# hku-mars/ImMesh

Hardware: AMD Instinct MI355X
Metric: scans/sec (reg+mesh), 100k-pt scan into 10M-voxel map (higher is better)
Workload: dtype f64

## Files before the change

### immesh_amd/csrc/c_api.cpp

```cpp
#include "host_ctx.hpp"
#include "imu_host.hpp"
#include <cmath>
#include <new>

#define RP_ABORTED 1
static thread_local std::string g_create_error;
thread_local KProf* g_kprof = nullptr;



extern "C" {

void immesh_default_config(immesh_config* c) {
    std::memset(c, 0, sizeof(*c));
    c->voxel_size = 0.5; c->max_layer = 2;
    for (int i = 0; i < 5; i++) c->layer_init[i] = 5;
    c->max_points_size = 100; c->planer_threshold = 0.01; c->dept_err = 0.02; c->beam_err = 0.05; c->calib_laser = 0;
    c->sigma_num = 3.0; c->max_iter = 4;
    c->extR[0] = c->extR[4] = c->extR[8] = 1.0;
    c->extT[0] = 0.04165; c->extT[1] = 0.02326; c->extT[2] = -0.0284;
    c->mesh_min_spacing = 0.1; c->mesh_voxel = 0.4; c->mesh_region = 10.0; c->mesh_append_budget = 10000;
}

const char* immesh_create_error(void) { return g_create_error.c_str(); }
// ... 195 lines not shown
        if (rc) { c->err = "all-reduce callback failed"; return IMMESH_E_INVAL; }
    }
    c->cnt.n_match += (int64_t)c->h_out48[RES_N_MATCH];
    c->cnt.n_plane_tests += (int64_t)c->h_out48[RES_PLANE_TESTS];
    c->cnt.n_extra_probe += (int64_t)c->h_out48[RES_EXTRA_PROBE];
    return 0;
}

static int fetch_matches(immesh_ctx* c, int n, std::vector<int8_t>& mt) {
    mt.resize(n);
    HIPCHK(c, hipMemcpyAsync(mt.data(), c->d_match, n, hipMemcpyDeviceToHost, c->stream));
    HIPCHK(c, hipStreamSynchronize(c->stream));
    return 0;
}

static int register_enqueue_chain(immesh_ctx* c, const float* d_pts, int n_ds, const imh::State& st) {
    RegIterArgs& a = c->reg_args;
    const int max_iter = c->cfg.max_iter;
    for (int it = 0; it < max_iter; it++) {
        a.it = it; a.mode = REG_MODE_SUMS;
        if (it == 0) {
            double p11[36];
            for (int r = 0; r < 6; r++) for (int q = 0; q < 6; q++) p11[r * 6 + q] = st.cov[r * 18 + q];
            if (!imh::invert(p11, a.mat, 6)) return singular_prior(c);
            for (int i = 0; i < 12; i++)
                for (int q = 0; q < 6; q++) { double sacc = 0; for (int k = 0; k < 6; k++) sacc += st.cov[(6 + i) * 18 + k] * a.mat[k * 6 + q]; a.mat[36 + i * 6 + q] = sacc; }
        }
        else if (it == 1) std::memcpy(a.mat, st.cov, sizeof(a.mat));
        launch_residual(c->stream, c->map, a, c->d_regstate, d_pts, n_ds, c->d_partials, c->d_done, c->d_out48, c->d_reg_out_host, c->reg_ticket, c->d_match, c->d_mnode,
                        c->d_dis, c->d_rinv, c->d_normal);
        if (c->rccl_comm) {
            const int rc = rccl_allreduce_f64(c, c->d_out48, RES_NV - 2, c->stream);
            if (rc) return rc;
        }
        launch_ekf_step(c->stream, a, c->d_regstate, c->d_out48, c->d_reg_out_host, c->reg_ticket);
    }
    return 0;
}
static int register_enqueue_fused(immesh_ctx* c, const float* d_pts, int n_ds, const imh::State& prior, const imh::State& st, const RpEpilogue* ep = nullptr) {
    const int max_iter = c->cfg.max_iter;
    RegIterArgs& a = c->reg_args;
    make_scan_params(c, st, st.cov, a.sp);
    a.max_iter = max_iter; a.pad = 0;
    if (c->tail_deferred && !c->rccl_comm) { a.pad = 1; c->tail_deferred = false; }
    else if (c->tail_deferred) { launch_map_update_tail(c->stream, c->map, c->d_counters_host); c->tail_deferred = false; }
    std::memcpy(a.st, st.R, 72); std::memcpy(a.st + 9, st.t, 24); std::memcpy(a.st + 12, st.vel, 24); std::memcpy(a.st + 15, st.bg, 24); std::memcpy(a.st + 18, st.ba, 24); std::memcpy(a.st + 21, st.g, 24);
    std::memcpy(a.prior, prior.R, 72); std::memcpy(a.prior + 9, prior.t, 24); std::memcpy(a.prior + 12, prior.vel, 24); std::memcpy(a.prior + 15, prior.bg, 24);
    std::memcpy(a.prior + 18, prior.ba, 24); std::memcpy(a.prior + 21, prior.g, 24);
    c->reg_ticket = (double)(++c->res_ticket);
    if (!c->rccl_comm) {
        a.mode = REG_MODE_FUSED; a.it = 0;
        if (c->knobs.rp_force_abort) a.pad |= 2;
        if (c->knobs.match_seq) a.pad |= 4;
        std::memcpy(a.mat, st.cov, sizeof(a.mat));
        const int par = (c->rp_parity ^= 1);
        RpEpilogue none{};
        launch_residual_persistent(c->stream, c->map, a, c->d_regstate, d_pts, n_ds, c->d_rp_slots[par], c->d_rp_slots[par ^ 1], c->d_counters_host, c->d_reg_out_host, c->reg_ticket, c->d_match, c->d_mnode,
                                   c->d_dis, c->d_rinv, c->d_normal, ep ? *ep : none, c->rp_max_blocks);
        return 0;
    }
    return register_enqueue_chain(c, d_pts, n_ds, st);
}
static int register_collect_fused(immesh_ctx* c, int n_ds, imh::State& st, int* n_iter, int* n_match, double* res_mean) {
    volatile double* flag = c->h_reg_out + REG_OUT_TICKET;
    const double ticket = c->reg_ticket;
    bool held;
    if (const int rc = wait_pinned(c, c->stream, [&] { return *flag == ticket; }, std::chrono::milliseconds(500), WAIT_NO_YIELD, &held)) return rc;
    if (c->prof.on) HIPCHK(c, hipStreamSynchronize(c->stream));
    if (!held) { c->err = "registration kernels did not complete"; return IMMESH_E_HIP; }
    const double* o = c->h_reg_out;
    if (o[REG_OUT_PASSES] < 0) return RP_ABORTED;
    imh::load_state(o + REG_OUT_STATE, st);
    const int iters = (int)o[REG_OUT_PASSES];
    if (n_iter) *n_iter = iters;
    if (n_match) *n_match = (int)o[REG_OUT_N_MATCH];
    if (res_mean) *res_mean = o[REG_OUT_N_MATCH] > 0 ? o[REG_OUT_SUM_DIS] / o[REG_OUT_N_MATCH] : 0.0;
    c->cnt.n_match += (int64_t)o[REG_OUT_N_MATCH_SUM];
    c->cnt.n_plane_tests += (int64_t)o[REG_OUT_PLANE_TESTS];
    c->cnt.n_extra_probe += (int64_t)o[REG_OUT_EXTRA_PROBE];
    c->cnt.n_iter += iters;
    c->cnt.n_ds = n_ds;
    c->last_n_ds = n_ds;
    return 0;
}
static int register_fallback_chain(immesh_ctx* c, const float* d_pts, int n_ds, const imh::State& st) {
    HIPCHK(c, hipStreamSynchronize(c->stream));
    c->rp_fallbacks++;
    c->reg_args.pad = 0;
    c->reg_ticket = (double)(++c->res_ticket);
    return register_enqueue_chain(c, d_pts, n_ds, st);
}
static bool use_fused_ekf(const immesh_ctx* c) {
    return !c->knobs.host_ekf && !c->allreduce && c->cfg.max_iter >= 2 && c->cfg.max_iter < 62 && (c->cfg.shard_world <= 1 || c->rccl_comm != nullptr);
}

static int register_device(immesh_ctx* c, const float* d_pts, int n_ds, const imh::State& prior, imh::State& st, int* n_iter, int* n_match, double* res_mean) {
    c->last_reg_pts = d_pts;
    if (use_fused_ekf(c)) {
        int rc = register_enqueue_fused(c, d_pts, n_ds, prior, st);
        if (rc) return rc;
        rc = register_collect_fused(c, n_ds, st, n_iter, n_match, res_mean);
        if (rc != RP_ABORTED) return rc;
        if ((rc = register_fallback_chain(c, d_pts, n_ds, st))) return rc;
        return register_collect_fused(c, n_ds, st, n_iter, n_match, res_mean);
    }
    imh::EkfLoop ekf;
// ... 336 lines not shown
    if (rc) return rc;
    for (int i = 0; i < 4; i++) ms[i] = c->timing[i];
    return 0;
}

int immesh_dump_planes(immesh_ctx* c, immesh_plane_rec* out, int64_t cap, int64_t* n_out) {
    if (!c || !n_out) return IMMESH_E_INVAL;
    (void)hipSetDevice(c->cfg.device);
    ProfBind _pb(c);
    if (const int s_rc = settle(c)) return s_rc;
    static_assert(sizeof(PlaneRecDev) == sizeof(immesh_plane_rec), "plane record layout");
    PlaneRecDev* d_out = nullptr;
    if (out && cap > 0) HIPCHK(c, hipMalloc((void**)&d_out, (size_t)cap * sizeof(PlaneRecDev)));
    launch_dump_planes(c->stream, c->map, d_out, d_out ? cap : 0, c->d_dump_count);
    unsigned long long cnt = 0;
    hipError_t e = hipMemcpyAsync(&cnt, c->d_dump_count, sizeof(cnt), hipMemcpyDeviceToHost, c->stream);
    if (e == hipSuccess) e = hipStreamSynchronize(c->stream);
    if (e == hipSuccess && d_out) e = hipMemcpy(out, d_out, (size_t)std::min<int64_t>(cap, (int64_t)cnt) * sizeof(PlaneRecDev), hipMemcpyDeviceToHost);
    if (d_out) (void)hipFree(d_out);
    if (e != hipSuccess) { c->err = std::string("dump_planes: ") + hipGetErrorString(e); return IMMESH_E_HIP; }
    *n_out = (int64_t)cnt;
    return 0;
}


int immesh_counters(immesh_ctx* c, immesh_counters_t* out, int32_t reset) {
    if (!c || !out) return IMMESH_E_INVAL;
    (void)hipSetDevice(c->cfg.device);
    ProfBind _pb(c);
    if (const int s_rc = settle(c)) return s_rc;
    int64_t stats[STATS_WORDS];
    HIPCHK(c, hipMemcpyAsync(stats, c->d_stats, sizeof(stats), hipMemcpyDeviceToHost, c->stream));
    HIPCHK(c, hipMemcpyAsync(c->h_counters, c->map.counters, 16 * sizeof(int32_t), hipMemcpyDeviceToHost, c->stream));
    HIPCHK(c, hipStreamSynchronize(c->stream));
    for (int k = 0; k < 64; k++) { stats[0] += stats[16 + k * 16]; stats[1] += stats[16 + k * 16 + 1]; }
    *out = c->cnt;
    out->n_refits = stats[0]; out->n_refit_pts = stats[1];
    out->n_root_voxels = c->h_counters[6]; out->n_nodes = c->h_counters[0];
    mesh_counters(c, out);
    if (c->reg_dbg) {
        unsigned long long t[64];
        HIPCHK(c, hipMemcpy(t, c->reg_dbg, sizeof(t), hipMemcpyDeviceToHost));
        if (!c->knobs.trace_file.empty()) {
            std::vector<unsigned long long> all(REG_DBG_WORDS);
            HIPCHK(c, hipMemcpy(all.data(), c->reg_dbg, all.size() * 8, hipMemcpyDeviceToHost));
            if (FILE* f = fopen(c->knobs.trace_file.c_str(), "wb")) { fwrite(all.data(), 8, all.size(), f); fclose(f); }
        }
        HIPCHK(c, hipMemset(c->reg_dbg, 0, sizeof(t)));
        fprintf(stderr, "[replay_list] slowest fast-path voxel %llu cycles (%llu pts), slowest general voxel %llu cycles (%llu pts); mean cycles fast %llu (%llu voxels) general %llu (%llu voxels); list gather + sort %llu per voxel\n",
                t[8] >> 16, t[8] & 0xFFFF, t[9] >> 16, t[9] & 0xFFFF, t[10] / std::max(1ull, t[12]), t[12], t[11] / std::max(1ull, t[13]), t[13], t[14] / std::max(1ull, t[12] + t[13]));
        const unsigned long long nwv = std::max(1ull, t[6]), npass = std::max(1ull, t[7]);
        fprintf(stderr, "[residual cycles of wavefront 0, %llu blocks x passes in %llu passes] prep %llu match %llu retry %llu hbuild %llu reduce %llu | last-block tail %llu per pass\n", t[6], t[7], t[0] / nwv, t[1] / nwv,
                t[2] / nwv, t[3] / nwv, t[4] / nwv, t[5] / npass);
    }
    if (reset) {
        mesh_counters_reset(c);
        std::memset(&c->cnt, 0, sizeof(c->cnt));
        HIPCHK(c, hipMemsetAsync(c->d_stats, 0, sizeof(stats), c->stream));
        HIPCHK(c, hipStreamSynchronize(c->stream));
    }
    return 0;
}

int immesh_forward_without_imu(const double* state_in, double dt, double cov_gyr, double cov_acc, double* state_out) {
    if (!state_in || !state_out) return IMMESH_E_INVAL;
    imh::State a, b;
    imh::load_state(state_in, a);
    imh::forward_without_imu(a, dt, cov_gyr, cov_acc, b);
    imh::store_state(b, state_out);
    return 0;
}

int immesh_set_allreduce(immesh_ctx* c, immesh_allreduce_fn fn, void* user) {
    if (!c) return IMMESH_E_INVAL;
    c->allreduce = fn; c->allreduce_user = user;
    return 0;
}

int immesh_shard_owner(const immesh_config* cfg, const int64_t* key3) {
    if (!cfg || !key3) return IMMESH_E_INVAL;
    if (cfg->shard_world <= 1) return 0;
    const int b = cfg->shard_brick_log2 > 0 ? cfg->shard_brick_log2 : 5;
    const int64_t bx = key3[0] >> b, by = key3[1] >> b, bz = key3[2] >> b;
    return imd::brick_owner(cfg->shard_scheme == 1 ? 1 : 0, cfg->shard_world, bx, by, bz, imd::pack_key(bx, by, bz));
}

int immesh_registration_fallbacks(immesh_ctx* c, int64_t* n) {
    if (!c || !n) return IMMESH_E_INVAL;
    *n = c->rp_fallbacks;
    return 0;
}

int immesh_profile_enable(immesh_ctx* c, int32_t on) {
    if (!c) return IMMESH_E_INVAL;
    mesh_wait_all(c);
    c->prof.on = on != 0;
    c->mesh_host.prof.on = on != 0;
    return 0;
}

int immesh_profile_read(immesh_ctx* c, immesh_kernel_stat* out, int32_t cap, int32_t* n_out, int32_t reset) {
    if (!c || !n_out) return IMMESH_E_INVAL;
    (void)hipSetDevice(c->cfg.device);
    if (c->stream) { HIPCHK(c, hipStreamSynchronize(c->stream)); c->prof.flush(); }
    mesh_wait_all(c);
    std::vector<std::string> names = c->prof.names;
// ... 17 lines not shown
```

### immesh_amd/csrc/host_knobs.hpp

```cpp
#pragma once
#include <hip/hip_runtime.h>
#include <algorithm>
#include <cstdlib>
#include <cstring>
#include <string>

struct Knobs {
    bool debug = false;
    bool debug_waits = false;
    std::string trace_file;
    int split_general = -1;
    bool no_priority = false;
    int mesh_cus = 0;
    int rp_blocks = 0;
    bool rp_force_abort = false;
    bool match_seq = false;
    bool host_ekf = false;
    bool serial_safe = false;
    bool serial_order = false;
    bool ds_radix = false;
    bool ds_no_gate = false;
    bool no_graph = false;
    int split_mode = 2;
    int mesh_room = 0;
    bool no_pipeline = false;
    int tri_stream = 1;
    int fused_wgs = 768;
    int list_div = 0;
    int mesh_grid_div = 1;

    static Knobs from_env(int mesh_npar) {
        auto on = [](const char* name) { return getenv(name) != nullptr; };
        auto num = [](const char* name, int unset) { const char* e = getenv(name); return e ? atoi(e) : unset; };
        Knobs k;
        k.debug = on("IMMESH_DEBUG"); k.debug_waits = on("IMMESH_DEBUG_WAITS");
        if (const char* e = getenv("IMMESH_TRACE_FILE")) k.trace_file = e;
        if (on("IMMESH_SPLIT_GENERAL")) k.split_general = num("IMMESH_SPLIT_GENERAL", 0);
        k.no_priority = on("IMMESH_NO_PRIORITY");
        k.mesh_cus = num("IMMESH_MESH_CUS", 0); if (k.mesh_cus < 8 || k.mesh_cus >= 1024) k.mesh_cus = 0;
        if (on("IMMESH_RP_BLOCKS")) k.rp_blocks = std::max(1, num("IMMESH_RP_BLOCKS", 0));
        k.rp_force_abort = on("IMMESH_RP_FORCE_ABORT"); k.match_seq = on("IMMESH_MATCH_SEQ"); k.host_ekf = on("IMMESH_HOST_EKF");
        k.serial_safe = on("IMMESH_SERIAL_SAFE"); k.serial_order = on("IMMESH_SERIAL_ORDER");
        k.ds_radix = on("IMMESH_DS_RADIX"); k.ds_no_gate = on("IMMESH_DS_NO_GATE");
        k.no_graph = on("IMMESH_NO_GRAPH");
        k.split_mode = on("IMMESH_NO_SPLIT") ? 0 : 2;
        if (on("IMMESH_SPLIT")) k.split_mode = num("IMMESH_SPLIT", 0) == 0 ? 0 : 1;
        if (on("IMMESH_MESH_ROOM")) k.mesh_room = std::min(std::max(num("IMMESH_MESH_ROOM", 0), 1), mesh_npar);
        k.no_pipeline = on("IMMESH_NO_PIPELINE");
        k.tri_stream = num("IMMESH_TRI_STREAM", 1);
        { const int v = num("IMMESH_FUSED_WGS", 0); k.fused_wgs = v >= 32 ? v : 768; }
        { const int v = num("IMMESH_LIST_DIV", 0); k.list_div = v >= 4 ? v : 0; }
        k.mesh_grid_div = std::max(1, num("IMMESH_MESH_GRID_DIV", 1));
        return k;
    }

    hipError_t make_stream(hipStream_t* s, int priority, bool maskable) const {
        if (!maskable || !mesh_cus) return hipStreamCreateWithPriority(s, hipStreamNonBlocking, priority);
        uint32_t mask[32];
        std::memset(mask, 0, sizeof(mask));
        for (int i = 0; i < mesh_cus; i++) mask[i >> 5] |= 1u << (i & 31);
        return hipExtStreamCreateWithCUMask(s, 32, mask);
    }
};
```

### immesh_amd/csrc/reg_kernels.hip

```cpp
#include <algorithm>
#include <cstdlib>
#include "regmap.hpp"
#include "kernels.hpp"
#include "prof.hpp"

using namespace imd;

struct PlaneRegs { double n[3], c[3], pv[21]; float d, radius; };
struct BestMatch { int node; int layer; double prob; bool ok; PlaneRegs P; };

IMD double plane_sigma(const double* pv, const double* J) {
    double tmp[6];
#pragma unroll
    for (int c = 0; c < 6; c++) {
        double s = 0;
#pragma unroll
        for (int r = 0; r < 6; r++) s += J[r] * pv[(r <= c) ? sym21_index(r, c) : sym21_index(c, r)];
        tmp[c] = s;
    }
    double sig = 0;
#pragma unroll
    for (int c = 0; c < 6; c++) sig += tmp[c] * J[c];
    return sig;
}
// ... 364 lines not shown
    const double passes = C[158] + 1.0;
    if (lane == 0) {
        dev_publish(&rs->tot[0], C[156]); dev_publish(&rs->tot[1], C[157]); dev_publish(&rs->tot[2], passes); dev_publish(&rs->tot[3], C[159]);
        __hip_atomic_store(&rs->rematch, rematch, __ATOMIC_RELAXED, __HIP_MEMORY_SCOPE_AGENT);
        __hip_atomic_store(&rs->done, stop ? 1 : 0, __ATOMIC_RELAXED, __HIP_MEMORY_SCOPE_AGENT);
        if (hist) { dev_publish(&hist[24], C[156]); dev_publish(&hist[25], C[157]); dev_publish(&hist[26], passes); dev_publish(&hist[27], C[159]); dev_publish(&hist[28], (double)rematch); dev_publish(&hist[29], stop ? 1.0 : 0.0); }
    }
    if (stop) {
        for (int e = lane; e < 324; e += 64) {
            const int r = e / 18, c = e % 18;
            double g6[6], c6[6];
#pragma unroll
            for (int k = 0; k < 6; k++) { g6[k] = W[108 + r * 6 + k]; c6[k] = cov[k * 18 + c]; }
            double sub = 0;
#pragma unroll
            for (int k = 0; k < 6; k++) sub += g6[k] * c6[k];
            const double sacc = cov[e] - sub;
            __hip_atomic_store((unsigned long long*)&reg_out[REG_OUT_COV + e], (unsigned long long)__double_as_longlong(sacc), __ATOMIC_RELAXED, __HIP_MEMORY_SCOPE_SYSTEM);
            if (r < 3 && c < 3) rs->sp.rot_var[r * 3 + c] = sacc;
            if (r >= 3 && r < 6 && c >= 3 && c < 6) rs->sp.t_var[(r - 3) * 3 + (c - 3)] = sacc;
        }
        if (lane < 24) {
            double v = 0;
#pragma unroll
            for (int k = 0; k < 24; k++) if (lane == k) v = st[k];
            __hip_atomic_store((unsigned long long*)&reg_out[REG_OUT_STATE + lane], (unsigned long long)__double_as_longlong(v), __ATOMIC_RELAXED, __HIP_MEMORY_SCOPE_SYSTEM);
        }
        if (lane == 0) {
            const double o[6] = {passes, n_match, res_sum, C[156], C[157], C[159]};
            for (int k = 0; k < 6; k++) __hip_atomic_store((unsigned long long*)&reg_out[REG_OUT_PASSES + k], (unsigned long long)__double_as_longlong(o[k]), __ATOMIC_RELAXED, __HIP_MEMORY_SCOPE_SYSTEM);
        }
        asm volatile("s_waitcnt vmcnt(0)" ::: "memory");
        __syncthreads();
        if (lane == 0) __hip_atomic_store(&reg_out[REG_OUT_TICKET], ticket, __ATOMIC_RELEASE, __HIP_MEMORY_SCOPE_SYSTEM);
    }
    EDBG(4);
    if (dbg && lane == 0) dbg[47] += 1;
#undef EDBG
    return stop;
}


#define RDBG(k) do { if (sp.dbg) { const unsigned long long _t = __builtin_readcyclecounter(); if (threadIdx.x == 0) atomicAdd(&sp.dbg[k], _t - tprev); tprev = _t; } } while (0)
__device__ __forceinline__ void map_update_tail(const RegMapDev& m, int32_t* __restrict__ host_counters) {
    const int np = m.counters[3];
    const int base = m.counters[2];
    for (int i = threadIdx.x; i < np; i += 256) m.free_ready[base + i] = m.free_pending[i];
    __syncthreads();
    if (threadIdx.x == 0) { m.counters[2] = base + np; m.counters[3] = 0; m.counters[7] = 0; m.counters[9] = 0; m.counters[10] = 0; m.counters[11] = 0; m.counters[12] = 0; }
    __syncthreads();
    if (threadIdx.x < 16) __hip_atomic_store(&host_counters[threadIdx.x], m.counters[threadIdx.x], __ATOMIC_RELAXED, __HIP_MEMORY_SCOPE_SYSTEM);
}

struct PointPrep {
    double pimu[3];
    double bcov[9];
    double b[9];
    double bv[9];
    unsigned long long key; int root;
    unsigned int slot;
};
#ifndef REG_UPD_PRIO
#define REG_UPD_PRIO 1
#endif
#define PREP_NO_KEY 0xFFFFFFFFFFFFFFFEull
#ifndef IMMESH_EPI_HINT
#define IMMESH_EPI_HINT 1
#endif
IMD void residual_prep(const ScanParams& sp, const float* __restrict__ pts, const int i, PointPrep& q) {
    const double p[3] = {(double)pts[(size_t)i * 3 + 0], (double)pts[(size_t)i * 3 + 1], (double)pts[(size_t)i * 3 + 2]};
    double pz[3] = {p[0], p[1], p[2]};
    if (pz[2] == 0) pz[2] = 0.001;
    calc_body_var(pz, sp.dept_err, sp.dvar_beam, q.bcov);
    double pimu_z[3];
    m3_vec(sp.extR, pz, pimu_z);
    pimu_z[0] += sp.extT[0]; pimu_z[1] += sp.extT[1]; pimu_z[2] += sp.extT[2];
    m3_vec(sp.extR, p, q.pimu);
    q.pimu[0] += sp.extT[0]; q.pimu[1] += sp.extT[1]; q.pimu[2] += sp.extT[2];
    {
        double cm[9], nc[9], nct[9], tmp[9];
        skew(pimu_z, cm);
#pragma unroll
        for (int k = 0; k < 9; k++) nc[k] = -cm[k];
#pragma unroll
        for (int r = 0; r < 3; r++)
#pragma unroll
            for (int c = 0; c < 3; c++) nct[r * 3 + c] = -cm[c * 3 + r];
        m3_mul(nc, sp.rot_var, tmp);
        m3_mul(tmp, nct, q.b);
    }
    double pthis[3] = {q.pimu[0], q.pimu[1], q.pimu[2]};
    calc_body_var(pthis, sp.dept_err, sp.calib_laser ? sp.dvar_calib : sp.dvar_beam, q.bv);
    q.key = PREP_NO_KEY; q.root = -1; q.slot = 0;
}
template <bool coop>
IMD void residual_pass(const RegMapDev& m, const ScanParams& sp, const double* Rm, const double* tv, const double* RextR, PointPrep& q, const int i, double* acc, unsigned long long& tprev,
                       int8_t* __restrict__ o_match, int32_t* __restrict__ o_node, float* __restrict__ o_dis, double* __restrict__ o_rinv, double* __restrict__ o_normal,
                       const bool active, unsigned int* __restrict__ wl) {
        const int lane = (int)(threadIdx.x & 63);
        double pwd[3];
        m3_vec(Rm, q.pimu, pwd);
        pwd[0] += tv[0]; pwd[1] += tv[1]; pwd[2] += tv[2];
        const double pw[3] = {(double)(float)pwd[0], (double)(float)pwd[1], (double)(float)pwd[2]};
        double var[9];
        {
            double a[9];
            m3_sandwich(Rm, q.bcov, a);
#pragma unroll
            for (int k = 0; k < 9; k++) var[k] = (a[k] + q.b[k]) + sp.t_var[k];
        }
        RDBG(0);
        float loc[3];
        int64_t kx[3];
#pragma unroll
        for (int j = 0; j < 3; j++) { loc[j] = loc_axis(pw[j] / m.voxel_size_d); kx[j] = (int64_t)loc[j]; }
        const bool mine = active && (m.shard_world <= 1 || shard_owner(m, kx[0], kx[1], kx[2]) == m.shard_rank);
        const uint64_t key = pack_key(kx[0], kx[1], kx[2]);
        int root = -1;
        if (mine) {
            if (key == q.key) root = q.root;
            else {
                const int64_t slot = hash_find(m, key);
                root = slot >= 0 ? m.htab[slot].root : -2;
                q.key = key; q.root = root; q.slot = (unsigned int)slot;
            }
        }
        BestMatch best; best.node = -1; best.layer = 0; best.prob = 0; best.ok = false;
        int n_tests = 0, n_extra = 0;
        int cur_root = (mine && root >= 0) ? root : -1;
        for (int round = 0; round < 2; round++) {
            bool is_tree = false;
            int tree_head = -1;
            if (cur_root >= 0) {
                if (!coop) match_tree(m, cur_root, pw, var, sp.sigma_num, best, n_tests);
                else {
                    const NodeRec& nr = m.nodes[cur_root];
                    const int flags = nr.flags, leaf_head = nr.leaf_head;
                    PlaneRegs P;
                    load_plane_geometry(nr, P);
                    load_plane_var(nr, P);
                    if (flags & NF_PLANE) {
                        n_tests++;
                        float dp, rd;
                        plane_gates(P, pw, dp, rd);
                        test_plane<false>(m, P, cur_root, 0, pw, var, sp.sigma_num, dp, rd, best);
                    } else if (m.max_layer > 0) { is_tree = true; tree_head = leaf_head; }
                }
            }
            if (coop && __any(is_tree)) match_trees_coop(m, is_tree, tree_head, pw, var, sp.sigma_num, best, n_tests, lane, wl);
            if (round == 0) {
                RDBG(1);
                const bool retry = mine && root >= 0 && !best.ok;
                cur_root = -1;
                if (retry) {
                    int64_t nk[3] = {kx[0], kx[1], kx[2]};
                    const float ql = m.nodes[root].quarter;
#pragma unroll
                    for (int j = 0; j < 3; j++) {
                        const double c = m.nodes[root].center[j];
                        if ((double)loc[j] > (c + (double)ql)) nk[j] = nk[j] + 1;
                        else if ((double)loc[j] < (c - (double)ql)) nk[j] = nk[j] - 1;
                    }
                    n_extra = 1;
                    const int64_t s2 = hash_find(m, pack_key(nk[0], nk[1], nk[2]));
                    if (s2 >= 0 && m.htab[s2].root >= 0) cur_root = m.htab[s2].root;
                }
                if (!__any(cur_root >= 0)) break;
            }
        }
        if (!active) return;
        RDBG(2);
        acc[29] += (double)n_tests; acc[30] += (double)n_extra;
        const bool matched = best.ok && best.node >= 0;
        o_match[i] = matched ? 1 : 0;
        o_node[i] = best.node;
        if (matched) {
            const PlaneRegs& P = best.P;
            const float nxf = (float)P.n[0], nyf = (float)P.n[1], nzf = (float)P.n[2];
            const float dis = (float)(pwd[0] * (double)nxf + pwd[1] * (double)nyf + pwd[2] * (double)nzf + (double)P.d);
            o_dis[i] = dis;
            o_normal[(size_t)i * 3 + 0] = P.n[0]; o_normal[(size_t)i * 3 + 1] = P.n[1]; o_normal[(size_t)i * 3 + 2] = P.n[2];
            const double nv[3] = {(double)nxf, (double)nyf, (double)nzf};
            double cm[9];
            skew(q.pimu, cm);
            double varw[9];
            m3_sandwich(RextR, q.bv, varw);
            const double J[6] = {pwd[0] - P.c[0], pwd[1] - P.c[1], pwd[2] - P.c[2], -P.n[0], -P.n[1], -P.n[2]};
            const double sigma_l = plane_sigma(P.pv, J);
            double vn[3];
            m3t_vec(varw, nv, vn);
            const double nvn = vn[0] * nv[0] + vn[1] * nv[1] + vn[2] * nv[2];
            const double ri = 1.0 / (sigma_l + nvn);
            o_rinv[i] = ri;
            double T1[9], A[3];
            m3_mul_bt(cm, Rm, T1);
            m3_vec(T1, nv, A);
            const double H[6] = {A[0], A[1], A[2], nv[0], nv[1], nv[2]};
            const double meas = -(double)dis;
            int k = 0;
#pragma unroll
            for (int r = 0; r < 6; r++) {
                const double hr = H[r] * ri;
#pragma unroll
                for (int c = r; c < 6; c++) acc[k++] += hr * H[c];
                acc[21 + r] += hr * meas;
            }
            acc[27] += 1.0;
            acc[28] += fabs((double)dis);
        }
}

template <bool COOP>
__global__ __launch_bounds__(64) void residual_kernel(RegMapDev m, RegIterArgs a, RegState* rs, const float* __restrict__ pts, int n,
                                                       double* __restrict__ partials, unsigned int* __restrict__ done_counter, double* __restrict__ out48,
                                                       double* __restrict__ reg_out, double ticket,
                                                       int8_t* __restrict__ o_match, int32_t* __restrict__ o_node,
                                                       float* __restrict__ o_dis, double* __restrict__ o_rinv, double* __restrict__ o_normal) {
    __builtin_amdgcn_s_setprio(3);
    const bool from_dev = a.mode == REG_MODE_SUMS && a.it > 0;
    if (from_dev && rs->done) return;
    ScanParams sp = a.sp;
    if (from_dev) {
#pragma unroll
        for (int k = 0; k < 9; k++) { sp.R[k] = rs->sp.R[k]; sp.RextR[k] = rs->sp.RextR[k]; sp.rot_var[k] = rs->sp.rot_var[k]; sp.t_var[k] = rs->sp.t_var[k]; }
#pragma unroll
        for (int k = 0; k < 3; k++) sp.t[k] = rs->sp.t[k];
    }
    const int i = blockIdx.x * blockDim.x + threadIdx.x;
    unsigned long long tprev = sp.dbg ? __builtin_readcyclecounter() : 0;
    if (sp.dbg && threadIdx.x == 0) { atomicAdd(&sp.dbg[6], 1ull); if (blockIdx.x == 0) atomicAdd(&sp.dbg[7], 1ull); }
    double acc[RES_NR];
#pragma unroll
    for (int k = 0; k < RES_NR; k++) acc[k] = 0;
    __shared__ double red[RES_NR][65];
    unsigned int* const coop_wl = (unsigned int*)&red[0][0];
    {
        PointPrep q = {};
        q.key = PREP_NO_KEY; q.root = -1;
        if (i < n) residual_prep(sp, pts, i, q);
        residual_pass<COOP>(m, sp, sp.R, sp.t, sp.RextR, q, i, acc, tprev, o_match, o_node, o_dis, o_rinv, o_normal, i < n, coop_wl);
    }
    RDBG(3);
    __builtin_amdgcn_fence(__ATOMIC_RELEASE, "workgroup"); __builtin_amdgcn_wave_barrier(); __builtin_amdgcn_fence(__ATOMIC_ACQUIRE, "workgroup");
    __shared__ int s_last;
    const int lane = threadIdx.x;
#pragma unroll
    for (int k = 0; k < RES_NR; k++) red[k][lane] = acc[k];
    __syncthreads();
    {
        const int k = lane & 31, half = lane >> 5;
        double ssum = 0;
        for (int j = 0; j < 32; j++) ssum += red[k][half * 32 + j];
        ssum += __shfl_xor(ssum, 32, 64);
        if (lane < RES_NR) __hip_atomic_store((unsigned long long*)&partials[(size_t)blockIdx.x * RES_NR + lane], (unsigned long long)__double_as_longlong(ssum), __ATOMIC_RELAXED, __HIP_MEMORY_SCOPE_AGENT);
    }
    asm volatile("s_waitcnt vmcnt(0)" ::: "memory");
    if (lane == 0) s_last = (atomicAdd(done_counter, 1u) == gridDim.x - 1) ? 1 : 0;
    __syncthreads();
    RDBG(4);
    if (!s_last) return;
    {
        const int k = lane & 31;
        const unsigned int nb = gridDim.x;
        double tot = 0;
        for (unsigned int b0 = (unsigned int)(lane >> 5); b0 < nb; b0 += 64) {
            double v[32];
#pragma unroll
            for (int u = 0; u < 32; u++) {
                const unsigned int b = b0 + 2u * u;
                v[u] = b < nb ? __longlong_as_double((long long)__hip_atomic_load((const unsigned long long*)&partials[(size_t)b * RES_NR + k], __ATOMIC_RELAXED, __HIP_MEMORY_SCOPE_AGENT)) : 0.0;
            }
#pragma unroll
            for (int u = 0; u < 32; u++) tot += v[u];
        }
        tot += __shfl_xor(tot, 32, 64);
        red[0][lane] = tot;
    }
    __syncthreads();
    double v48 = 0;
    if (lane < 36) { const int r = lane / 6, c = lane % 6; v48 = red[0][r <= c ? sym21_index(r, c) : sym21_index(c, r)]; }
    else if (lane < 42) v48 = red[0][21 + (lane - 36)];
    else if (lane < 46) v48 = red[0][27 + (lane - 42)];
    if (lane == 0) *done_counter = 0;
    if (lane < RES_NV - 1) __hip_atomic_store((unsigned long long*)&out48[lane], (unsigned long long)__double_as_longlong(v48), __ATOMIC_RELAXED, __HIP_MEMORY_SCOPE_SYSTEM);
    asm volatile("s_waitcnt vmcnt(0)" ::: "memory");
    RDBG(5);
    if (lane == 0 && a.mode == REG_MODE_HOST) __hip_atomic_store(&out48[RES_TICKET], ticket, __ATOMIC_RELEASE, __HIP_MEMORY_SCOPE_SYSTEM);
}

#define RP_MAX_BLOCKS 128
#define RP_SPIN_TICKS 100000000ull
static_assert(COOP_WORDS * 4 <= RES_NR * 65 * 8, "the cooperative matcher's scratch lives in a wavefront's reduction transpose buffer");
struct RpShared {
    double red[4][RES_NR][65];
    double wsum[4][RES_NR];
    double pc[108];
    double st[24];
    double prior[24];
    double sums[48];
    double X[36], y[6], sol[18];
    double M[108], XM[108];
    double tot[4];
    int rematch, stop;
};
IMD void lds_wave_sync() {
    __builtin_amdgcn_fence(__ATOMIC_RELEASE, "workgroup");
    __builtin_amdgcn_wave_barrier();
    __builtin_amdgcn_fence(__ATOMIC_ACQUIRE, "workgroup");
}
__device__ __forceinline__ void rp_prior_minus_state(const RpShared& S, double* __restrict__ R12, double* __restrict__ vec6) {
#pragma unroll
    for (int k = 0; k < 12; k++) R12[k] = S.st[k];
    double Rt[9], rotd[9], pR[9];
#pragma unroll
    for (int k = 0; k < 9; k++) pR[k] = S.prior[k];
#pragma unroll
    for (int i = 0; i < 3; i++)
#pragma unroll
        for (int j2 = 0; j2 < 3; j2++) Rt[i * 3 + j2] = R12[j2 * 3 + i];
    m3_mul(Rt, pR, rotd);
    dev_so3_log(rotd, vec6);
#pragma unroll
    for (int k = 0; k < 3; k++) vec6[3 + k] = S.prior[9 + k] - R12[9 + k];
}
__device__ __forceinline__ void rp_update(RpShared& S, const RegIterArgs& a, const int it, const int lane, const bool writer, const double* __restrict__ R12,
                                          const double* __restrict__ vec6, unsigned long long* dbg) {
    unsigned long long tk = dbg ? __builtin_readcyclecounter() : 0;
#define EDBG(k) do { if (dbg) { const unsigned long long _t = __builtin_readcyclecounter(); if (lane == 0 && writer) dbg[40 + (k)] += _t - tk; tk = _t; } } while (0)
    const int own = lane < 18 ? lane : 0;
    const int row = (lane >= 6 && lane < 12) ? lane - 6 : 0;
    double hrow[6], trow[6];
#pragma unroll
    for (int c = 0; c < 6; c++) { hrow[c] = S.sums[row * 6 + c]; trow[c] = S.pc[36 + (own >= 6 ? own - 6 : 0) * 6 + c]; }
    const double hz = S.sums[RES_HTZ + row];
    const double st_own = S.st[own + 6], prior_own = S.prior[own + 6];
    double w[6];
    {
        double sacc = 0;
#pragma unroll
        for (int c = 0; c < 6; c++) sacc += hrow[c] * vec6[c];
        const double wl = hz - sacc;
#pragma unroll
        for (int c = 0; c < 6; c++) w[c] = rl_d(wl, 6 + c);
    }
    double c6[6];
    {
        const int j = lane < 12 ? lane : 0;
#pragma unroll
        for (int r = 0; r < 6; r++) c6[r] = j < 6 ? S.sums[r * 6 + j] + S.pc[r * 6 + j] : ((r == j - 6) ? 1.0 : 0.0);
#pragma unroll
        for (int col = 0; col < 6; col++) {
            const double d = rl_d(c6[col], col);
            double f[6];
#pragma unroll
            for (int r = 0; r < 6; r++) f[r] = rl_d(c6[r], col);
            c6[col] = c6[col] * fast_rcp(d);
// ... 133 lines not shown
    }
    const int G = (int)gridDim.x - 1;
    if ((int)blockIdx.x == G) {
        if (a.pad & 1) map_update_tail(m, host_counters);
        __threadfence();
        __syncthreads();
        if (threadIdx.x == 0) dev_publish(&slots[RP_TAIL_WORD], 1.0);
        return;
    }
    if (wv == 0) {
        double c6[6], trw[2][6];
        const int j = lane < 12 ? lane : 0;
#pragma unroll
        for (int r = 0; r < 6; r++) c6[r] = j < 6 ? a.mat[r * 18 + j] : ((r == j - 6) ? 1.0 : 0.0);
#pragma unroll
        for (int h = 0; h < 2; h++) {
            const int e = lane + 64 * h, i = e < 72 ? e / 6 : 0;
#pragma unroll
            for (int k = 0; k < 6; k++) trw[h][k] = a.mat[(6 + i) * 18 + k];
        }
        const double st_l = a.st[lane < 24 ? lane : 0], prior_l = a.prior[lane < 24 ? lane : 0];
#pragma unroll
        for (int col = 0; col < 6; col++) {
            const double d = rl_d(c6[col], col);
            double f[6];
#pragma unroll
            for (int r = 0; r < 6; r++) f[r] = rl_d(c6[r], col);
            c6[col] = c6[col] * fast_rcp(d);
#pragma unroll
            for (int r = 0; r < 6; r++) if (r != col) c6[r] -= f[r] * c6[col];
        }
        if (lane >= 6 && lane < 12) {
#pragma unroll
            for (int r = 0; r < 6; r++) S.pc[r * 6 + (lane - 6)] = c6[r];
        }
        lds_wave_sync();
#pragma unroll
        for (int h = 0; h < 2; h++) {
            const int e = lane + 64 * h;
            if (e < 72) {
                const int q = e % 6;
                double sacc = 0;
#pragma unroll
                for (int k = 0; k < 6; k++) sacc += trw[h][k] * S.pc[k * 6 + q];
                S.pc[36 + e] = sacc;
            }
        }
        if (lane < 24) { S.st[lane] = st_l; S.prior[lane] = prior_l; }
        if (lane == 0) { S.rematch = 0; S.stop = 0; S.tot[0] = S.tot[1] = S.tot[2] = S.tot[3] = 0.0; }
    }
    __syncthreads();
    const int ntiles = (n + 63) / 64;
    const bool one_tile = ntiles <= G * 4;
    PointPrep prep = {};
    prep.key = PREP_NO_KEY; prep.root = -1;
    for (int it = 0; it < a.max_iter; it++) {
        unsigned long long* const tr = (sp.dbg && threadIdx.x == 0 && it < 8) ? sp.dbg + (64 + 16384 * 8) + ((size_t)it * 512 + blockIdx.x) * 8 : nullptr;
        if (tr) {
            tr[0] = __builtin_amdgcn_s_memrealtime();
            if (it == 0) tr[4] = t_entry;
            if (it == 1) { tr[4] = (unsigned long long)__builtin_amdgcn_s_getreg((4) | (0 << 6) | (31 << 11)); tr[5] = (unsigned long long)__builtin_amdgcn_s_getreg((20) | (0 << 6) | (31 << 11)); }
        }
        if (sp.dbg && threadIdx.x == 0) { atomicAdd(&sp.dbg[6], 1ull); if (blockIdx.x == 0) atomicAdd(&sp.dbg[7], 1ull); }
        double Rm[9], tv[3], RextR[9];
#pragma unroll
        for (int k = 0; k < 9; k++) Rm[k] = uni_d(S.st[k]);
#pragma unroll
        for (int k = 0; k < 3; k++) tv[k] = uni_d(S.st[9 + k]);
        {
            double t9[9];
            m3_mul(Rm, sp.extR, t9);
#pragma unroll
            for (int k = 0; k < 9; k++) RextR[k] = uni_d(t9[k]);
        }
        if (sp.dbg) tprev = __builtin_readcyclecounter();
        double acc[RES_NR];
#pragma unroll
        for (int k = 0; k < RES_NR; k++) acc[k] = 0;
        for (int tile = blockIdx.x * 4 + wv; tile < ntiles; tile += G * 4) {
            const int i = tile * 64 + lane;
            if (i < n && !(one_tile && it > 0)) residual_prep(sp, pts, i, prep);
            residual_pass<COOP>(m, sp, Rm, tv, RextR, prep, i, acc, tprev, o_match, o_node, o_dis, o_rinv, o_normal, i < n, (unsigned int*)&S.red[wv][0][0]);
        }
        RDBG(3);
#pragma unroll
        for (int k = 0; k < RES_NR; k++) S.red[wv][k][lane] = acc[k];
        lds_wave_sync();
        {
            const int k = lane & 31, half = lane >> 5;
            double ssum = 0;
            for (int j = 0; j < 32; j++) ssum += S.red[wv][k][half * 32 + j];
            ssum += __shfl_xor(ssum, 32, 64);
            if (lane < RES_NR) S.wsum[wv][lane] = ssum;
        }
        __syncthreads();
        double* const pass_slots = slots + (size_t)it * RP_MAX_BLOCKS * RES_NR;
        if (wv == 0) {
            if (lane < RES_NR) dev_publish(&pass_slots[(size_t)blockIdx.x * RES_NR + lane], ((S.wsum[0][lane] + S.wsum[1][lane]) + S.wsum[2][lane]) + S.wsum[3][lane]);
            RDBG(4);
            if (tr) tr[1] = __builtin_amdgcn_s_memrealtime();
            const int k = lane & 31;
            double tot = 0;
            double R12[12], vec6[6];
            bool have_vec = false;
            __builtin_amdgcn_s_setprio(1);
            bool aborted = false;
            unsigned long long spin_t0 = 0;
            unsigned int spins = 0;
            for (int b0 = lane >> 5; b0 < G && !aborted; b0 += 64) {
                double v[32];
                for (;;) {
                    unsigned long long bits[32];
#pragma unroll
                    for (int u = 0; u < 32; u++) {
                        const int b = b0 + 2 * u;
                        bits[u] = 0;
                        if (b < G) bits[u] = __hip_atomic_load((const unsigned long long*)&pass_slots[(size_t)b * RES_NR + k], __ATOMIC_RELAXED, __HIP_MEMORY_SCOPE_AGENT);
                    }
                    unsigned long long tailbits = 0;
                    if (it == 0) tailbits = __hip_atomic_load((const unsigned long long*)&slots[RP_TAIL_WORD], __ATOMIC_RELAXED, __HIP_MEMORY_SCOPE_AGENT);
                    const unsigned long long abortbits = __hip_atomic_load((const unsigned long long*)&slots[RP_ABORT_WORD], __ATOMIC_RELAXED, __HIP_MEMORY_SCOPE_AGENT);
                    if (!have_vec) { rp_prior_minus_state(S, R12, vec6); have_vec = true; }
                    bool ok = tailbits != RP_SLOT_SENTINEL;
#pragma unroll
                    for (int u = 0; u < 32; u++) { ok = ok && bits[u] != RP_SLOT_SENTINEL; v[u] = __longlong_as_double((long long)bits[u]); }
                    if (__any(abortbits != RP_SLOT_SENTINEL) || (a.pad & 2)) { aborted = true; break; }
                    if (__all(ok)) break;
                    if ((++spins & 63u) == 0) {
                        const unsigned long long now = __builtin_amdgcn_s_memrealtime();
                        if (spin_t0 == 0) spin_t0 = now;
                        else if (now - spin_t0 > RP_SPIN_TICKS) { aborted = true; break; }
                    }
                    __builtin_amdgcn_s_sleep(1);
                }
#pragma unroll
// ... 1254 lines not shown
```

Before: 5981.

## Cache per-point plane geometry and neighbour lookup in LDS across registration passes

After: 6000, median of 4. No clear change (+0.3%).

```diff
diff --git a/immesh_amd/csrc/c_api.cpp b/immesh_amd/csrc/c_api.cpp
--- a/immesh_amd/csrc/c_api.cpp
+++ b/immesh_amd/csrc/c_api.cpp
@@ -271,6 +271,7 @@
         a.mode = REG_MODE_FUSED; a.it = 0;
         if (c->knobs.rp_force_abort) a.pad |= 2;
         if (c->knobs.match_seq) a.pad |= 4;
+        if (!c->knobs.plane_cache) a.pad |= 8;
         std::memcpy(a.mat, st.cov, sizeof(a.mat));
         const int par = (c->rp_parity ^= 1);
         RpEpilogue none{};
@@ -713,6 +714,8 @@
         const unsigned long long nwv = std::max(1ull, t[6]), npass = std::max(1ull, t[7]);
         fprintf(stderr, "[residual cycles of wavefront 0, %llu blocks x passes in %llu passes] prep %llu match %llu retry %llu hbuild %llu reduce %llu | last-block tail %llu per pass\n", t[6], t[7], t[0] / nwv, t[1] / nwv,
                 t[2] / nwv, t[3] / nwv, t[4] / nwv, t[5] / npass);
+        fprintf(stderr, "[residual match / retry by pass, cycles of wavefront 0] pass 0: match %llu retry %llu (%llu blocks) | passes >= 1: match %llu retry %llu (%llu blocks x passes)\n", t[48] / std::max(1ull, t[52]),
+                t[49] / std::max(1ull, t[52]), t[52], t[50] / std::max(1ull, t[53]), t[51] / std::max(1ull, t[53]), t[53]);
     }
     if (reset) {
         mesh_counters_reset(c);
diff --git a/immesh_amd/csrc/host_knobs.hpp b/immesh_amd/csrc/host_knobs.hpp
--- a/immesh_amd/csrc/host_knobs.hpp
+++ b/immesh_amd/csrc/host_knobs.hpp
@@ -15,6 +15,7 @@
     int rp_blocks = 0;
     bool rp_force_abort = false;
     bool match_seq = false;
+    bool plane_cache = true;
     bool host_ekf = false;
     bool serial_safe = false;
     bool serial_order = false;
@@ -40,6 +41,7 @@
         k.mesh_cus = num("IMMESH_MESH_CUS", 0); if (k.mesh_cus < 8 || k.mesh_cus >= 1024) k.mesh_cus = 0;
         if (on("IMMESH_RP_BLOCKS")) k.rp_blocks = std::max(1, num("IMMESH_RP_BLOCKS", 0));
         k.rp_force_abort = on("IMMESH_RP_FORCE_ABORT"); k.match_seq = on("IMMESH_MATCH_SEQ"); k.host_ekf = on("IMMESH_HOST_EKF");
+        k.plane_cache = num("IMMESH_PLANE_CACHE", 1) != 0;
         k.serial_safe = on("IMMESH_SERIAL_SAFE"); k.serial_order = on("IMMESH_SERIAL_ORDER");
         k.ds_radix = on("IMMESH_DS_RADIX"); k.ds_no_gate = on("IMMESH_DS_NO_GATE");
         k.no_graph = on("IMMESH_NO_GRAPH");
diff --git a/immesh_amd/csrc/reg_kernels.hip b/immesh_amd/csrc/reg_kernels.hip
--- a/immesh_amd/csrc/reg_kernels.hip
+++ b/immesh_amd/csrc/reg_kernels.hip
@@ -440,6 +440,7 @@
     if (threadIdx.x < 16) __hip_atomic_store(&host_counters[threadIdx.x], m.counters[threadIdx.x], __ATOMIC_RELAXED, __HIP_MEMORY_SCOPE_SYSTEM);
 }
 
+#define PREP_NO_KEY 0xFFFFFFFFFFFFFFFEull
 struct PointPrep {
     double pimu[3];
     double bcov[9];
@@ -448,13 +449,37 @@
     unsigned long long key; int root;
     unsigned int slot;
 };
+#define PCACHE_SLOTS 34
+struct PlaneCache {
+    double* col;
+    IMD int* words() const { return (int*)&col[33 * 256]; }
+    IMD unsigned long long& nkey() const { return *(unsigned long long*)&col[32 * 256]; }
+    IMD int& geo_root() const { return ((int*)&col[31 * 256])[1]; }
+    IMD void reset() const { if (col) { words()[0] = -1; words()[1] = -1; nkey() = PREP_NO_KEY; geo_root() = -1; } }
+};
+#define RDBG_BY_PASS(k) do { if (sp.dbg) { const unsigned long long _t = __builtin_readcyclecounter(); if (threadIdx.x == 0) { atomicAdd(&sp.dbg[k], _t - tprev); \
+        atomicAdd(&sp.dbg[48 + (pass > 0 ? 2 : 0) + ((k) - 1)], _t - tprev); } tprev = _t; } } while (0)
 #ifndef REG_UPD_PRIO
 #define REG_UPD_PRIO 1
 #endif
-#define PREP_NO_KEY 0xFFFFFFFFFFFFFFFEull
 #ifndef IMMESH_EPI_HINT
 #define IMMESH_EPI_HINT 1
 #endif
+IMD void pcache_load(const PlaneCache pc, PlaneRegs& P) {
+#pragma unroll
+    for (int k = 0; k < 3; k++) { P.n[k] = pc.col[k * 256]; P.c[k] = pc.col[(3 + k) * 256]; }
+#pragma unroll
+    for (int k = 0; k < 21; k++) P.pv[k] = pc.col[(6 + k) * 256];
+    const double dr = pc.col[27 * 256];
+    P.d = __int_as_float(__double2loint(dr)); P.radius = __int_as_float(__double2hiint(dr));
+}
+IMD void pcache_store(const PlaneCache pc, const PlaneRegs& P) {
+#pragma unroll
+    for (int k = 0; k < 3; k++) { pc.col[k * 256] = P.n[k]; pc.col[(3 + k) * 256] = P.c[k]; }
+#pragma unroll
+    for (int k = 0; k < 21; k++) pc.col[(6 + k) * 256] = P.pv[k];
+    pc.col[27 * 256] = __hiloint2double(__float_as_int(P.radius), __float_as_int(P.d));
+}
 IMD void residual_prep(const ScanParams& sp, const float* __restrict__ pts, const int i, PointPrep& q) {
     const double p[3] = {(double)pts[(size_t)i * 3 + 0], (double)pts[(size_t)i * 3 + 1], (double)pts[(size_t)i * 3 + 2]};
     double pz[3] = {p[0], p[1], p[2]};
@@ -484,7 +509,7 @@
 template <bool coop>
 IMD void residual_pass(const RegMapDev& m, const ScanParams& sp, const double* Rm, const double* tv, const double* RextR, PointPrep& q, const int i, double* acc, unsigned long long& tprev,
                        int8_t* __restrict__ o_match, int32_t* __restrict__ o_node, float* __restrict__ o_dis, double* __restrict__ o_rinv, double* __restrict__ o_normal,
-                       const bool active, unsigned int* __restrict__ wl) {
+                       const bool active, unsigned int* __restrict__ wl, const PlaneCache pc = PlaneCache{nullptr}, const int pass = 0, const double* __restrict__ bv_col = nullptr) {
         const int lane = (int)(threadIdx.x & 63);
         double pwd[3];
         m3_vec(Rm, q.pimu, pwd);
@@ -516,6 +541,7 @@
         BestMatch best; best.node = -1; best.layer = 0; best.prob = 0; best.ok = false;
         int n_tests = 0, n_extra = 0;
         int cur_root = (mine && root >= 0) ? root : -1;
+        const bool own_cached = coop && pc.col && cur_root >= 0 && cur_root == pc.words()[0];
         for (int round = 0; round < 2; round++) {
             bool is_tree = false;
             int tree_head = -1;
@@ -523,10 +549,15 @@
                 if (!coop) match_tree(m, cur_root, pw, var, sp.sigma_num, best, n_tests);
                 else {
                     const NodeRec& nr = m.nodes[cur_root];
-                    const int flags = nr.flags, leaf_head = nr.leaf_head;
+                    int flags = NF_PLANE, leaf_head = -1;
                     PlaneRegs P;
-                    load_plane_geometry(nr, P);
-                    load_plane_var(nr, P);
+                    if (own_cached && round == 0) pcache_load(pc, P);
+                    else {
+                        flags = nr.flags; leaf_head = nr.leaf_head;
+                        load_plane_geometry(nr, P);
+                        load_plane_var(nr, P);
+                        if (pc.col && round == 0 && (flags & NF_PLANE)) { pcache_store(pc, P); pc.words()[0] = cur_root; }
+                    }
                     if (flags & NF_PLANE) {
                         n_tests++;
                         float dp, rd;
@@ -537,27 +568,41 @@
             }
             if (coop && __any(is_tree)) match_trees_coop(m, is_tree, tree_head, pw, var, sp.sigma_num, best, n_tests, lane, wl);
             if (round == 0) {
-                RDBG(1);
+                RDBG_BY_PASS(1);
                 const bool retry = mine && root >= 0 && !best.ok;
                 cur_root = -1;
                 if (retry) {
                     int64_t nk[3] = {kx[0], kx[1], kx[2]};
-                    const float ql = m.nodes[root].quarter;
+                    const bool geo_cached = pc.col && root == pc.geo_root();
+                    const float ql = geo_cached ? __int_as_float(__double2loint(pc.col[31 * 256])) : m.nodes[root].quarter;
+                    double ctr[3];
+#pragma unroll
+                    for (int j = 0; j < 3; j++) ctr[j] = geo_cached ? pc.col[(28 + j) * 256] : m.nodes[root].center[j];
+                    if (pc.col && !geo_cached) {
+#pragma unroll
+                        for (int j = 0; j < 3; j++) pc.col[(28 + j) * 256] = ctr[j];
+                        pc.col[31 * 256] = __hiloint2double(root, __float_as_int(ql));
+                    }
 #pragma unroll
                     for (int j = 0; j < 3; j++) {
-                        const double c = m.nodes[root].center[j];
+                        const double c = ctr[j];
                         if ((double)loc[j] > (c + (double)ql)) nk[j] = nk[j] + 1;
                         else if ((double)loc[j] < (c - (double)ql)) nk[j] = nk[j] - 1;
                     }
                     n_extra = 1;
-                    const int64_t s2 = hash_find(m, pack_key(nk[0], nk[1], nk[2]));
-                    if (s2 >= 0 && m.htab[s2].root >= 0) cur_root = m.htab[s2].root;
+                    const uint64_t nkey = pack_key(nk[0], nk[1], nk[2]);
+                    if (pc.col && nkey == pc.nkey()) cur_root = pc.words()[1];
+                    else {
+                        const int64_t s2 = hash_find(m, nkey);
+                        if (s2 >= 0 && m.htab[s2].root >= 0) cur_root = m.htab[s2].root;
+                        if (pc.col) { pc.nkey() = nkey; pc.words()[1] = cur_root; }
+                    }
                 }
                 if (!__any(cur_root >= 0)) break;
             }
         }
         if (!active) return;
-        RDBG(2);
+        RDBG_BY_PASS(2);
         acc[29] += (double)n_tests; acc[30] += (double)n_extra;
         const bool matched = best.ok && best.node >= 0;
         o_match[i] = matched ? 1 : 0;
@@ -571,8 +616,10 @@
             const double nv[3] = {(double)nxf, (double)nyf, (double)nzf};
             double cm[9];
             skew(q.pimu, cm);
-            double varw[9];
-            m3_sandwich(RextR, q.bv, varw);
+            double varw[9], bv[9];
+#pragma unroll
+            for (int k = 0; k < 9; k++) bv[k] = bv_col ? bv_col[k * 256] : q.bv[k];
+            m3_sandwich(RextR, bv, varw);
             const double J[6] = {pwd[0] - P.c[0], pwd[1] - P.c[1], pwd[2] - P.c[2], -P.n[0], -P.n[1], -P.n[2]};
             const double sigma_l = plane_sigma(P.pv, J);
             double vn[3];
@@ -616,7 +663,7 @@
     }
     const int i = blockIdx.x * blockDim.x + threadIdx.x;
     unsigned long long tprev = sp.dbg ? __builtin_readcyclecounter() : 0;
-    if (sp.dbg && threadIdx.x == 0) { atomicAdd(&sp.dbg[6], 1ull); if (blockIdx.x == 0) atomicAdd(&sp.dbg[7], 1ull); }
+    if (sp.dbg && threadIdx.x == 0) { atomicAdd(&sp.dbg[6], 1ull); atomicAdd(&sp.dbg[a.it > 0 ? 53 : 52], 1ull); if (blockIdx.x == 0) atomicAdd(&sp.dbg[7], 1ull); }
     double acc[RES_NR];
 #pragma unroll
     for (int k = 0; k < RES_NR; k++) acc[k] = 0;
@@ -626,7 +673,7 @@
         PointPrep q = {};
         q.key = PREP_NO_KEY; q.root = -1;
         if (i < n) residual_prep(sp, pts, i, q);
-        residual_pass<COOP>(m, sp, sp.R, sp.t, sp.RextR, q, i, acc, tprev, o_match, o_node, o_dis, o_rinv, o_normal, i < n, coop_wl);
+        residual_pass<COOP>(m, sp, sp.R, sp.t, sp.RextR, q, i, acc, tprev, o_match, o_node, o_dis, o_rinv, o_normal, i < n, coop_wl, PlaneCache{nullptr}, a.it);
     }
     RDBG(3);
     __builtin_amdgcn_fence(__ATOMIC_RELEASE, "workgroup"); __builtin_amdgcn_wave_barrier(); __builtin_amdgcn_fence(__ATOMIC_ACQUIRE, "workgroup");
@@ -690,6 +737,8 @@
     double M[108], XM[108];
     double tot[4];
     int rematch, stop;
+    double pcache[PCACHE_SLOTS][256];
+    double bv[9][256];
 };
 IMD void lds_wave_sync() {
     __builtin_amdgcn_fence(__ATOMIC_RELEASE, "workgroup");
@@ -929,8 +978,11 @@
     __syncthreads();
     const int ntiles = (n + 63) / 64;
     const bool one_tile = ntiles <= G * 4;
+    const bool keep_on_chip = one_tile && !(a.pad & 8);
+    const PlaneCache pcache{keep_on_chip ? &S.pcache[0][threadIdx.x] : nullptr};
     PointPrep prep = {};
     prep.key = PREP_NO_KEY; prep.root = -1;
+    pcache.reset();
     for (int it = 0; it < a.max_iter; it++) {
         unsigned long long* const tr = (sp.dbg && threadIdx.x == 0 && it < 8) ? sp.dbg + (64 + 16384 * 8) + ((size_t)it * 512 + blockIdx.x) * 8 : nullptr;
         if (tr) {
@@ -938,7 +990,7 @@
             if (it == 0) tr[4] = t_entry;
             if (it == 1) { tr[4] = (unsigned long long)__builtin_amdgcn_s_getreg((4) | (0 << 6) | (31 << 11)); tr[5] = (unsigned long long)__builtin_amdgcn_s_getreg((20) | (0 << 6) | (31 << 11)); }
         }
-        if (sp.dbg && threadIdx.x == 0) { atomicAdd(&sp.dbg[6], 1ull); if (blockIdx.x == 0) atomicAdd(&sp.dbg[7], 1ull); }
+        if (sp.dbg && threadIdx.x == 0) { atomicAdd(&sp.dbg[6], 1ull); atomicAdd(&sp.dbg[it > 0 ? 53 : 52], 1ull); if (blockIdx.x == 0) atomicAdd(&sp.dbg[7], 1ull); }
         double Rm[9], tv[3], RextR[9];
 #pragma unroll
         for (int k = 0; k < 9; k++) Rm[k] = uni_d(S.st[k]);
@@ -956,8 +1008,12 @@
         for (int k = 0; k < RES_NR; k++) acc[k] = 0;
         for (int tile = blockIdx.x * 4 + wv; tile < ntiles; tile += G * 4) {
             const int i = tile * 64 + lane;
-            if (i < n && !(one_tile && it > 0)) residual_prep(sp, pts, i, prep);
-            residual_pass<COOP>(m, sp, Rm, tv, RextR, prep, i, acc, tprev, o_match, o_node, o_dis, o_rinv, o_normal, i < n, (unsigned int*)&S.red[wv][0][0]);
+            if (i < n && !(one_tile && it > 0)) {
+                residual_prep(sp, pts, i, prep);
+#pragma unroll
+                for (int k = 0; k < 9; k++) S.bv[k][threadIdx.x] = prep.bv[k];
+            }
+            residual_pass<COOP>(m, sp, Rm, tv, RextR, prep, i, acc, tprev, o_match, o_node, o_dis, o_rinv, o_normal, i < n, (unsigned int*)&S.red[wv][0][0], pcache, it, &S.bv[0][threadIdx.x]);
         }
         RDBG(3);
 #pragma unroll
```
